# Stanford-ILIAD/PantheonRL

Measured on AMD Instinct MI355X. Metric: env-steps/sec (all agents) Overcooked-simple PPO self-play, higher is better.
Workload: dtype f32; 1 GPU; OvercookedMultiEnv-v0 layout=simple, PPO self-play (two independent PPO learners per GPU), synthetic (n_envs, n_steps, obs_dim) rollouts; n_envs=1024, n_steps=128, obs_dim=62, features=62, n_logits=6, batch_size=32768, n_epochs=10, agents_per_gpu=2, parallelism=2 agent(s) per gpu x1 gpu(s) = 2 learners (single process), launch_mode=graph, gemm_mode=2, action_masks=none, rollout=scripted, rollout_requested=scripted

## Files before the change

### include/pantheon_hip.h

```cpp
#ifndef PANTHEON_HIP_H
#define PANTHEON_HIP_H

#ifdef __cplusplus
extern "C" {
#endif

#define PH_ABI_VERSION 7
#define PH_HIDDEN 64
#define PH_MAX_COMP 256
#define PH_MAX_LOGITS 64
#define PH_MAX_BOX_ACT 16
#define PH_NSTAT 8
#define PH_MOD_MAX 8
#define PH_MAX_RANKS 16

#define PH_SPACE_BOX 0
#define PH_SPACE_DISCRETE 1

typedef struct ph_ctx ph_ctx;

typedef struct ph_space {
  int kind;
  int n;
  int nvec[PH_MAX_COMP];
// ... 30 lines not shown
  float clip_range;
  float clip_range_vf;
  float ent_coef;
  float vf_coef;
  float max_grad_norm;
  float target_kl;
  int normalize_advantage;
  float adam_beta1, adam_beta2, adam_eps;
} ph_ppo_hyper;

typedef struct ph_opt_state {
  float *params;
  float *adam_m;
  float *adam_v;
  int *step;
} ph_opt_state;

int ph_abi_version(void);
const char *ph_last_error(void);
int ph_device_count(int *n_out );
int ph_ctx_create(int device, ph_ctx **out );
int ph_ctx_destroy(ph_ctx *ctx);
int ph_ctx_set_stream(ph_ctx *ctx, void *hip_stream );
int ph_ctx_sync(ph_ctx *ctx);
int ph_graph_begin(ph_ctx *ctx);
int ph_graph_end(ph_ctx *ctx, int *graph_id_out );
int ph_graph_launch(ph_ctx *ctx, int graph_id);
int ph_ctx_set_rng_epoch(ph_ctx *ctx, unsigned long long *epoch_dev );
int ph_rng_epoch_advance(ph_ctx *ctx);
int ph_debug_set_profile_buffer(ph_ctx *ctx, long long *stamps_dev);
int ph_debug_weight_image_mismatches(ph_ctx *ctx, const ph_spec *spec, const float *params, int *mismatches);
int ph_set_exclusive_device(ph_ctx *ctx, int exclusive);
int ph_ctx_step_errors(ph_ctx *ctx, unsigned int *count_out );
int ph_timer_start(ph_ctx *ctx);
int ph_timer_stop(ph_ctx *ctx, float *ms_out );

int ph_layout_of(const ph_spec *spec , ph_layout *out );
int ph_debug_split_tables(const ph_spec *spec, int *slab_map, int *image_map, int *eligible);
int ph_debug_split_oh_tables(const ph_spec *spec, int *slab_map, int *image_map, int *slab_len_out, int *image_elems_out,
                             int *eligible);

int ph_buffer_add(ph_ctx *ctx, const ph_spec *spec, const ph_rollout *rb, int pos, const float *obs ,
                  const float *actions , const float *episode_start ,
                  const float *values , const float *log_probs );
int ph_buffer_add_reward(ph_ctx *ctx, const ph_rollout *rb, int pos, const float *reward ,
                         const unsigned char *env_mask );
int ph_buffer_add_reward_const(ph_ctx *ctx, const ph_rollout *rb, int pos, float reward);
#define PH_JOINT_MATCH_BONUS 0
#define PH_JOINT_RPS 1
int ph_ctx_set_joint_reward_rule(ph_ctx *ctx, int rule);

int ph_buffer_add_reward_joint(ph_ctx *ctx, const ph_rollout *rb, int pos, const float *base_reward ,
                               const int *joint_actions, int n_seats, int seat, const int *partner_seat ,
                               float bonus);
int ph_roundrobin_env_step(ph_ctx *ctx, const int *joint_actions, int *partnerid, const float *base_reward,
                           const float *done, float *reward_out, int *alt_action_out, float *next_block, int block_ld,
                           int n_partners, float bonus, int n);
typedef struct ph_rr_link {
  int n_partners, rank;
  int n, block_ld;
  void *area[PH_MAX_RANKS];
  unsigned long long *error;
  unsigned long long timeout_cycles;
} ph_rr_link;
typedef struct ph_rr_ego {
  const ph_spec *spec;
// ... 563 lines not shown
```

### pantheonrl_amd/_native.py

```python
from __future__ import annotations

import ctypes as C
import os
from typing import Optional, Sequence

PH_HIDDEN = 64
PH_MAX_COMP = 256
PH_MAX_LOGITS = 64
PH_MAX_BOX_ACT = 16
PH_NSTAT = 8
PH_SPACE_BOX = 0
PH_SPACE_DISCRETE = 1
STAT_NAMES = ("policy_loss", "value_loss", "entropy_loss", "clip_fraction", "approx_kl", "loss", "grad_norm", "applied")

_HERE = os.path.dirname(os.path.abspath(__file__))
LIB_PATH = os.environ.get("PANTHEON_HIP_LIB") or os.path.join(_HERE, "csrc", "libpantheon_hip.so")


class NativeError(RuntimeError):
    """Raised for any non-zero status from the C ABI (message from ph_last_error)."""


class PhSpace(C.Structure):
    _fields_ = [("kind", C.c_int), ("n", C.c_int), ("nvec", C.c_int * PH_MAX_COMP)]
# ... 238 lines not shown


SIGNATURES = {
    "ph_abi_version": [],
    "ph_roundrobin_env_step": [_vp, _vp, _vp, _vp, _vp, _vp, _vp, _vp, _i, _i, C.c_float, _i],
    "ph_last_error": [],
    "ph_device_count": [C.POINTER(_i)],
    "ph_ctx_create": [_i, C.POINTER(_vp)],
    "ph_ctx_destroy": [_vp],
    "ph_ctx_set_stream": [_vp, _vp],
    "ph_ctx_sync": [_vp],
    "ph_graph_begin": [_vp],
    "ph_graph_end": [_vp, C.POINTER(_i)],
    "ph_graph_launch": [_vp, _i],
    "ph_ctx_set_rng_epoch": [_vp, _vp],
    "ph_rng_epoch_advance": [_vp],
    "ph_debug_set_profile_buffer": [_vp, _vp],
    "ph_set_exclusive_device": [_vp, _i],
    "ph_ctx_step_errors": [_vp, C.POINTER(C.c_uint)],
    "ph_debug_weight_image_mismatches": [_vp, C.POINTER(PhSpec), _vp, C.POINTER(C.c_int)],
    "ph_timer_start": [_vp],
    "ph_timer_stop": [_vp, C.POINTER(C.c_float)],
    "ph_layout_of": [C.POINTER(PhSpec), C.POINTER(PhLayout)],
    "ph_debug_split_tables": [C.POINTER(PhSpec), C.POINTER(C.c_int), C.POINTER(C.c_int), C.POINTER(C.c_int)],
    "ph_debug_split_oh_tables": [C.POINTER(PhSpec), _vp, _vp, C.POINTER(_i), C.POINTER(_i), C.POINTER(_i)],
    "ph_buffer_add": [_vp, C.POINTER(PhSpec), C.POINTER(PhRollout), _i, _vp, _vp, _vp, _vp, _vp],
    "ph_buffer_add_reward": [_vp, C.POINTER(PhRollout), _i, _vp, _vp],
    "ph_buffer_add_reward_joint": [_vp, C.POINTER(PhRollout), _i, _vp, _vp, _i, _i, _vp, C.c_float],
    "ph_buffer_reset": [_vp, C.POINTER(PhSpec), C.POINTER(PhRollout)],
    "ph_gae": [_vp, C.POINTER(PhRollout), _vp, _vp, _d, _d, _i],
    "ph_policy_forward": [_vp, C.POINTER(PhSpec), _vp, _vp, _i, _vp, _vp, _vp, _ull, _ull, _i, _vp, _vp, _vp, _vp, _vp,
                          _vp, C.POINTER(PhRollout), _i, _vp, _vp, _i],
    "ph_ctx_set_joint_reward_rule": [_vp, _i],
    "ph_adapmult_layout_of": [C.POINTER(PhSpec), _i, _vp],
    "ph_adapmult_forward": [_vp, C.POINTER(PhSpec), _i, _vp, _vp, _i, _vp, _vp, _vp, _ull, _ull, _i, _vp, _vp, _vp, _vp, _vp,
                            _vp, C.POINTER(PhRollout), _i, _vp],
    "ph_adapmult_minibatch_grad": [_vp, C.POINTER(PhSpec), _i, _vp, C.POINTER(PhRollout), C.POINTER(PhPpoHyper), _vp, _i, _vp, _vp,
                                   _vp],
    "ph_adapmult_train": [_vp, C.POINTER(PhSpec), _i, C.POINTER(PhOptState), C.POINTER(PhRollout), C.POINTER(PhPpoHyper), _i, _i,
                          _vp, _ull, _vp, _vp],
    "ph_policy_act_host": [_vp, C.POINTER(PhSpec), _vp, _vp, _i, _vp, _ull, _ull, _i, _vp, _vp, _vp, C.POINTER(PhRollout), _i, _i],
    "ph_buffer_add_reward_const": [_vp, C.POINTER(PhRollout), _i, C.c_float],
    "ph_policy_step_multi": [_vp, _i, C.POINTER(PhStepCall)],
    "ph_policy_forward_ragged": [_vp, C.POINTER(PhSpec), _vp, _vp, _vp, _ull, _ull, _i, _vp, _vp, _vp, C.POINTER(PhRollout),
                                 _vp, _vp, _vp],
    "ph_buffer_add_reward_ragged": [_vp, C.POINTER(PhRollout), _vp, _vp, _vp],
    "ph_ragged_advance": [_vp, C.POINTER(PhRollout), _vp, _vp],
    "ph_buffer_compact_columns": [_vp, C.POINTER(PhSpec), C.POINTER(PhRollout), C.POINTER(PhRollout), _vp, _i],
    "ph_fix_illegal_actions": [_vp, _vp, _vp, _i, _i],
    "ph_rps_step": [_vp, _vp, _vp, _vp, _vp, _i],
    "ph_liar_step": [_vp, _vp, _vp, _vp, _vp, _vp, _vp, _vp, _vp, _vp, _i],
    "ph_liar_reset": [_vp, _vp, _vp, _vp, _vp, _vp, _ull, _ull, C.c_float, _i],
    "ph_liar_obs": [_vp, _vp, _vp, _vp, _vp, _vp, _vp, _i],
    "ph_liar_selfplay_step": [_vp, C.POINTER(PhLiarSelfPlay), _i, _ull, _i],
    "ph_liar_selfplay_rollout": [_vp, C.POINTER(PhLiarSelfPlay), _i, _i, _ull],
    "ph_pool_forward": [_vp, C.POINTER(PhSpec), C.POINTER(PhPoolMember), _i, _vp, _vp, _vp, _ull, _vp, _vp, _i],
    "ph_liar_default_actions": [_vp, _vp, _vp, _vp, _i],
    "ph_liar_pool_step": [_vp, C.POINTER(PhLiarPool), _i, _ull, _i],
    "ph_liar_xplay_step": [_vp, C.POINTER(PhLiarXplay), _ull, _i],
    "ph_xplay_stats": [_vp, _vp, _vp, _vp, _i, _i, _i, _vp],
    "ph_episode_stats": [_vp, C.POINTER(PhEpisodeScan)],
    "ph_liar_record_attach": [_vp, C.POINTER(PhLiarRecord)],
    "ph_liar_record_export": [_vp, C.POINTER(PhLiarRecord), _i, _vp, _vp, _vp, C.c_longlong],
    "ph_block_reset": [_vp, _i, _vp, _vp, _ull, _ull, _i],
    "ph_block_step": [_vp, _i, _vp, _vp, _i, _vp, _vp, _vp, _vp, _i],
    "ph_block_obs": [_vp, _i, _vp, _i, _vp, _vp, _i],
# ... 172 lines not shown
def adapmult_layout_of(spec: PhSpec, context_size: int) -> PhAdapMultLayout:
    lay = PhAdapMultLayout()
    check(load().ph_adapmult_layout_of(C.byref(spec), int(context_size), C.byref(lay)))
    return lay


def ptr(t) -> Optional[int]:
    if t is None:
        return None
    return t.data_ptr()


class Context:

    def __init__(self, device_index: int = 0):
        self.lib = load()
        h = C.c_void_p()
        check(self.lib.ph_ctx_create(int(device_index), C.byref(h)))
        self.handle = h
        self.device_index = int(device_index)
        self.exclusive_hint = False

    def set_stream(self, raw_stream: int) -> None:
        if raw_stream != getattr(self, "_bound_stream", None):
            check(self.lib.ph_ctx_set_stream(self.handle, C.c_void_p(raw_stream)))
            self._bound_stream = raw_stream

    def sync(self) -> None:
        check(self.lib.ph_ctx_sync(self.handle))

    def set_joint_reward_rule(self, rule: str) -> None:
        check(self.lib.ph_ctx_set_joint_reward_rule(self.handle, {"match": 0, "rps": 1}[rule]))

    def step_errors(self) -> int:
        n = C.c_uint(0)
        check(self.lib.ph_ctx_step_errors(self.handle, C.byref(n)))
        return int(n.value)

    def set_exclusive_device(self, exclusive: bool) -> None:
        check(self.lib.ph_set_exclusive_device(self.handle, int(bool(exclusive))))
        self.exclusive_hint = bool(exclusive)

    def close(self) -> None:
        if getattr(self, "handle", None):
            self.lib.ph_ctx_destroy(self.handle)
            self.handle = None

    def __del__(self):
        try:
            self.close()
        except Exception:
            pass


def feistel_indices(n: int, perm_seed: int, epoch: int, start: int = 0, count: Optional[int] = None):
    import numpy as np
    count = n - start if count is None else count
    out = (C.c_int * count)()
    check(load().ph_feistel_indices(int(n), int(perm_seed), int(epoch), int(start), int(count), out))
    return np.frombuffer(out, dtype=np.int32).copy()


def env_space_of(observation_space) -> PhSpace:
    kind = type(observation_space).__name__
    if kind == "Box":
        import numpy as np
# ... 51 lines not shown
```

### pantheonrl_amd/csrc/ph_abi.hip

```cpp
#include <dlfcn.h>
#include <hip/hip_runtime.h>
#include <rccl/rccl.h>

#include <atomic>
#include <chrono>
#include <cmath>
#include <cstdio>
#include <cstdint>
#include <cstring>
#include <mutex>
#include <string>
#include <vector>

#include "ph_launch.h"
#include "ph_block.h"
#include "ph_arch.h"
#include "ph_pool.h"
#include "ph_xplay.h"
#include "ph_record.h"
#include "ph_episode.h"
#include "ph_adap_vec.h"

namespace ph {

// ... 124 lines not shown
  float* am_buf = nullptr;
  size_t am_buf_cap = 0;
  float* adap_extra = nullptr;
  size_t adap_extra_cap = 0;
  float* adap_loss = nullptr;
  size_t adap_loss_cap = 0;
  float* scalars = nullptr;
  int* stop_flag = nullptr;
  std::vector<SpecCache> specs;
  std::vector<hipGraphExec_t> graphs;
  bool capturing = false;
  hipEvent_t ev0 = nullptr, ev1 = nullptr;
  ph_p2p* p2p_dev = nullptr;
  ph_p2p p2p_host;
  bool p2p_valid = false;
  void* comm = nullptr;
  int comm_world = 1, comm_rank = 0;
  hipEvent_t ev_grad = nullptr;
  int num_cu = 256;
  int exchange_blocks_per_cu = 0;
  unsigned long long* rng_epoch = nullptr;
  ph::RecordLog rec{};
  bool recording = false;
  ph::PoolMemberDev* pool_dev = nullptr;
  ph::PoolMemberDev pool_host[PH_MAX_POOL];
  int pool_count = 0;
  bool pool_wide = false;
  size_t pool_tower_lds = 0;
  int* pool_order = nullptr;
  size_t pool_order_cap = 0;
  int* pool_tiles = nullptr;
  size_t pool_tiles_cap = 0;
  long long* prof = nullptr;
  double* ep_partial = nullptr;
  size_t ep_partial_cap = 0;
  unsigned int* ep_ticket = nullptr;
  struct ModWs {
    float* act = nullptr;
    size_t act_cap = 0;
    int* maps = nullptr;
    ph_spec spec;
    ph_modular mod;
    bool maps_valid = false;
    float* kl_sum = nullptr;
    int* scratch = nullptr;
  } mw;
};

namespace {

struct DevGuard {
  int prev = -1;
  bool switched = false;
  explicit DevGuard(const ph_ctx* ctx) {
    if (!ctx) return;
    if (hipGetDevice(&prev) == hipSuccess && prev != ctx->device) switched = hipSetDevice(ctx->device) == hipSuccess;
  }
  ~DevGuard() {
    if (switched) (void)hipSetDevice(prev);
  }
  DevGuard(const DevGuard&) = delete;
  DevGuard& operator=(const DevGuard&) = delete;
};

template <typename T>
int ensure(const ph_ctx* ctx, T*& p, size_t& cap, size_t n) {
// ... 270 lines not shown
  a.prof = ctx->prof;
  a.deterministic = deterministic;
  fwd_bind_bases(a, rb, episode_start_in, pos_env, record_mask);
  PH_HIP(arch ? ph::launch_arch_fwd(a, ad, gemm_mode, ctx->stream) : ph::launch_policy_fwd(a, gemm_mode, ctx->stream));
  return 0;
}

int scripted_rollout_run(const char* who, ph_ctx* ctx, const ph_spec* spec, const ph_arch* arch, const float* params,
                         const float* obs_seq, const float* rew_seq, const float* done_seq, int n, int n_steps,
                         const float* episode_start0, unsigned long long seed, unsigned long long counter0, int* actions_i32,
                         float* values, float* log_probs, const ph_rollout* rb, int pos0, int gemm_mode) {
  if (!ctx) return fail("null ctx");
  if (!params || !obs_seq || !rew_seq || !done_seq || !episode_start0) return fail_who(who, ": null argument");
  if ((uintptr_t)params % 16 != 0) return fail_who(who, ": params must be 16-byte aligned");
  if (n <= 0 || n_steps <= 0) return fail_who(who, ": n and n_steps must be positive");
  if (check_rb(rb)) return 1;
  if (n != rb->E) return fail_who(who, ": n must equal the rollout buffer's E");
  if (pos0 < 0 || pos0 > rb->T - n_steps) return fail_who(who, ": rows pos0 .. pos0 + n_steps - 1 must lie in the buffer");
  ph::FwdArgs a;
  ph::ArchDims ad;
  if (fwd_args(a, ctx, spec, false, params, obs_seq, n, seed, counter0, actions_i32, values, log_probs, arch, &ad)) return 1;
  if (!arch && !ph::fwd16_eligible(a.nd, n))
    return fail_who(who, ": needs the 16-row forward's shape class (one feature chunk, one Discrete head of <= 8 logits, "
                         "n < 16384); use ph_policy_forward per step");
  a.prof = ctx->prof;
  if (fwd_bind_row(who, a, rb, pos0, episode_start0, nullptr)) return 1;
  ph::ScriptedSteps sc;
  std::memset(&sc, 0, sizeof(sc));
  sc.n_steps = n_steps;
  sc.obs_seq = obs_seq;
  sc.rew_seq = rew_seq;
  sc.done_seq = done_seq;
  PH_HIP(arch ? ph::launch_arch_rollout(a, ad, sc, gemm_mode, ctx->stream)
              : ph::launch_policy_fwd16_rollout(a, sc, gemm_mode, ctx->stream));
  return 0;
}

ph::AdvStatArgs adv_args_epochs(const ph_ctx* ctx, const ph_rollout* rb, const int* perms, unsigned long long perm_seed, int batch,
                                int n_mb) {
  const int N = rb->T * rb->E;
  ph::AdvStatArgs aa{};
  aa.rb_adv = rb->advantages;
  aa.T = rb->T;
  aa.E = rb->E;
  aa.perms = perms;
  aa.perm_n = (uint32_t)N;
  aa.perm_hb = ph::feistel_half_bits((uint32_t)N);
  aa.perm_seed = perm_seed;
  aa.epoch = ctx->rng_epoch;
  aa.N = N;
  aa.batch = batch;
  aa.n_mb = n_mb;
  aa.out = ctx->advstats;
  aa.partial = ctx->advpart;
  aa.idx_out = perms ? nullptr : ctx->perm_idx;
  aa.phys_out = ctx->perm_phys;
  return aa;
}
ph::AdvStatArgs adv_args_minibatch(const ph_ctx* ctx, const ph_rollout* rb, const int* indices, int nb) {
  ph::AdvStatArgs aa{};
  aa.rb_adv = rb->advantages;
  aa.T = rb->T;
  aa.E = rb->E;
  aa.perms = indices;
  aa.perm_hb = 1;
  aa.N = nb;
  aa.batch = nb;
// ... 150 lines not shown
}

int ph_ctx_destroy(ph_ctx* ctx) {
  DevGuard dev_guard(ctx);
  if (!ctx) return 0;
  (void)hipStreamSynchronize(ctx->stream);
  for (auto g : ctx->graphs)
    if (g) (void)hipGraphExecDestroy(g);
  for (auto& s : ctx->specs) {
    if (s.obs_off) (void)hipFree(s.obs_off);
    if (s.slab_map) (void)hipFree(s.slab_map);
    if (s.slab_map_split) (void)hipFree(s.slab_map_split);
    if (s.wimage_map) (void)hipFree(s.wimage_map);
    if (s.act_off) (void)hipFree(s.act_off);
  }
  void* ptrs[] = {ctx->wimage, ctx->mw.act, ctx->mw.maps, ctx->mw.kl_sum, ctx->mw.scratch, ctx->advpart, ctx->p2p_dev, ctx->slabs, ctx->statpart, ctx->grad, ctx->blocksq, ctx->advstats, ctx->adam_bias, ctx->perm_idx, ctx->perm_phys, ctx->ximg, ctx->rec_pi, ctx->rec_vf, ctx->rowrec, ctx->step_words, ctx->step_gen, ctx->scalars, ctx->stop_flag,
                  ctx->adap_extra, ctx->adap_loss, ctx->am_buf, ctx->pool_dev, ctx->pool_order, ctx->pool_tiles, ctx->ep_partial, ctx->ep_ticket};
  for (void* p : ptrs)
    if (p) (void)hipFree(p);
  if (ctx->act_stage_host) (void)hipHostFree(ctx->act_stage_host);
  if (ctx->act_done_host) (void)hipHostFree(ctx->act_done_host);
  if (ctx->ev0) (void)hipEventDestroy(ctx->ev0);
  if (ctx->ev1) (void)hipEventDestroy(ctx->ev1);
  if (ctx->ev_grad) (void)hipEventDestroy(ctx->ev_grad);
  (void)ph_comm_destroy(ctx);
  delete ctx;
  return 0;
}

int ph_ctx_set_joint_reward_rule(ph_ctx* ctx, int rule) {
  if (!ctx) return fail("null ctx");
  if (rule != PH_JOINT_MATCH_BONUS && rule != PH_JOINT_RPS) return fail("ph_ctx_set_joint_reward_rule: unknown rule");
  ctx->joint_reward_rule = rule;
  return 0;
}

int ph_ctx_set_stream(ph_ctx* ctx, void* hip_stream) {
  DevGuard dev_guard(ctx);
  if (!ctx) return fail("null ctx");
  ctx->stream = (hipStream_t)hip_stream;
  return 0;
}

int ph_ctx_sync(ph_ctx* ctx) {
  DevGuard dev_guard(ctx);
  if (!ctx) return fail("null ctx");
  PH_HIP(hipStreamSynchronize(ctx->stream));
  return 0;
}

int ph_graph_begin(ph_ctx* ctx) {
  DevGuard dev_guard(ctx);
  if (!ctx) return fail("null ctx");
  if (ctx->capturing) return fail("already capturing");
  if (ctx->stream == nullptr) return fail("graph capture needs a non-default stream (ph_ctx_set_stream)");
  PH_HIP(hipStreamBeginCapture(ctx->stream, hipStreamCaptureModeRelaxed));
  ctx->capturing = true;
  return 0;
}

int ph_graph_end(ph_ctx* ctx, int* graph_id_out) {
  DevGuard dev_guard(ctx);
  if (!ctx || !graph_id_out) return fail("null ctx/graph_id_out");
  if (!ctx->capturing) return fail("not capturing");
  ctx->capturing = false;
  hipGraph_t g = nullptr;
// ... 3076 lines not shown
```

### pantheonrl_amd/csrc/ph_launch.h

```cpp
#pragma once
#include "ph_device.h"

namespace ph {

__host__ __device__ inline unsigned p2p_stamp32(unsigned long long epoch, int T, int t) {
  return (unsigned)(epoch * (unsigned long long)T + (unsigned long long)t + 1ull);
}

__device__ __forceinline__ void p2p_note_timeout(unsigned long long* error, int kind, int t, unsigned long long index,
                                                 unsigned long long want, unsigned long long seen) {
  if (atomicAdd(error, 1ull) == 0ull) {
    error[1] = (unsigned long long)(unsigned)kind | ((unsigned long long)(unsigned)(t & 0xffffff) << 8) | (index << 32);
    error[2] = want;
    error[3] = seen;
  }
}

__device__ __forceinline__ void poll_backoff(int& polls) {
  if (polls < 16) __builtin_amdgcn_s_sleep(2);
  else if (polls < 64) __builtin_amdgcn_s_sleep(16);
  else __builtin_amdgcn_s_sleep(127);
  ++polls;
}

// ... 40 lines not shown
  const int* partner_seat;
  float bonus;
  int reward_rule;
  const unsigned char* env_mask;
  unsigned int* host_done;
  unsigned int host_seq;
};

struct ScriptedSteps {
  int n_steps;
  const float* obs_seq;
  const float* rew_seq;
  const float* done_seq;
  const unsigned char* mask_seq;
  int mask_policy, mask_env;
};

constexpr int MAX_LOCAL_AGENTS = 4;
struct P2PStep {
  const ph_p2p* x;
  int t;
  int a_local;
  int persistent;
};
__host__ __device__ inline int p2p_persistent_slot(unsigned long long epoch, int T, int t) { return (int)(epoch & 1ull) * T + t; }
struct FwdMulti {
  FwdArgs a[MAX_LOCAL_AGENTS];
  P2PStep px;
};
struct ScriptedMulti {
  ScriptedSteps sc[MAX_LOCAL_AGENTS];
};
bool fwd16_eligible(const NetDims& nd, int n);
hipError_t launch_policy_fwd16_rollout(const FwdArgs& a, const ScriptedSteps& sc, int gemm_mode, hipStream_t s);
hipError_t launch_policy_fwd16_exchange_rollout(const FwdMulti& m, const ScriptedMulti& sm, int n_agents, hipStream_t s);
hipError_t exchange_rollout_blocks_per_cu(int* blocks_out);

struct GradArgs {
  NetDims nd;
  const float* params;
  const float* rb_obs;
  const float* rb_act;
  const float* rb_val;
  const float* rb_logp;
  const float* rb_adv;
  const float* rb_ret;
  int T, E;
  const int* idx;
  const int* idx_phys;
  uint32_t perm_n, perm_hb;
  uint64_t perm_seed;
  int perm_epoch;
  const unsigned long long* epoch;
  int mb_start;
  int nb;
  const float* advstats;
  float clip, clip_vf, ent_coef, vf_coef;
  int norm_adv;
  float* slabs;
  float* statpart;
  const int* stop_flag;
  long long* prof;
  int ntiles;
  const unsigned short* wimage;
  const uint4* ximg;
  int ximg_zero_row;
  const uint4* rec_pi;
// ... 391 lines not shown
```

### pantheonrl_amd/csrc/ph_policy.hip

```cpp
#include <cstring>
#include <initializer_list>
#include "ph_rowtail.h"
#include "ph_liar_group.h"
#include "ph_pool.h"
#include "ph_bc_row.h"

namespace ph {


template <int R, int LP, bool VALU>
__device__ __forceinline__ void policy_fwd_body(const FwdArgs& a) {
  extern __shared__ __attribute__((aligned(16))) float smem[];
  constexpr int NT = R * 4;
  const NetDims& nd = a.nd;
  constexpr int Lp = LP, LDO = LP + 1;
  float* bufA = smem;
  float* bufB = bufA + R * LDH;
  float* w1s = bufB + R * LDH;
  float* w2s = w1s + HID * LDH;
  float* wos = w2s + HID * LDH;
  float* outs = wos + HID * LDO;
  float* b1s = outs + R * LDO;
  float* b2s = b1s + HID;
  float* bos = b2s + HID;
// ... 182 lines not shown
  __builtin_assume(a.rb_val != nullptr);
  __builtin_assume(a.rb_logp != nullptr);
  __builtin_assume(a.es_in != nullptr);
}
bool fwd_args_lean(const FwdArgs& a, bool joint_ok = false) {
  static int enabled = -1;
  if (enabled < 0) {
    const char* e = getenv("PH_ROLLOUT_LEAN");
    enabled = (e && e[0] == '0') ? 0 : 1;
  }
#ifdef PH_LEAN_PROF
  constexpr bool lean_prof = true;
#else
  constexpr bool lean_prof = false;
#endif
  return enabled && !a.mask && !a.uniforms && !a.given_actions && !a.deterministic && !a.act_f32 && !a.entropy && !a.logits && (lean_prof || !a.prof) &&
         !a.pos_env && !a.rec_mask && (joint_ok || (!a.joint && !a.joint_ll)) && !a.env_mask && !a.host_done && a.rb_obs && a.rb_act && a.rb_rew &&
         a.rb_es && a.rb_val && a.rb_logp && a.es_in;
}

constexpr int ZS_FLOATS = 4 * 16 * 8;

struct TailWaveHook {
  bool arrive, alive;
  long long* stamp;
  __device__ __forceinline__ void split(int act, float lse) const {
    if (stamp) stamp[4] = (long long)clock64();
    if (arrive) asm volatile("s_waitcnt lgkmcnt(0)\n\ts_barrier" ::"v"(act), "v"(lse) : "memory");
    else asm volatile("" ::"v"(act), "v"(lse));
  }
  __device__ __forceinline__ bool live() const { return alive; }
};

template <bool VALU, int LEAN = 0, int TW = 0>
__device__ __forceinline__ void policy_fwd16_body(const FwdArgs& a0, const ph_p2p* px = nullptr, int px_t = 0, int px_a_local = 0,
                                                  int agent = 0, const ScriptedSteps* sc = nullptr, int px_persistent = 0) {
  extern __shared__ __attribute__((aligned(16))) float smem[];
  constexpr int R = 16, NT = 256;
  const NetDims& nd = a0.nd;
  FwdArgs a = a0;
  if constexpr (LEAN == 1) fwd_args_pin_lean<false>(a);
  if constexpr (LEAN == 2) fwd_args_pin_lean<true>(a);
  if constexpr (TW != 0) {
    a.mask = nullptr;
    a.env_mask = nullptr;
    a.uniforms = nullptr;
    a.given_actions = nullptr;
    a.deterministic = 0;
  }
#ifdef PH_LEAN_PROF
  long long* const prof0 = a0.prof;
#else
  long long* const prof0 = LEAN ? nullptr : a0.prof;
#endif
  float* xs = smem;
  float* hs = xs + R * LDH;
  float* zs = hs + R * LDH;
  int* rowphys = (int*)(zs + ZS_FLOATS);
  float* upre = (float*)(rowphys + 16);
  unsigned long long** pxll = (unsigned long long**)(upre + 32);

  const int tid = threadIdx.x;
  const int wave = TW ? __builtin_amdgcn_readfirstlane(tid >> 6) : tid >> 6, lane = tid & 63, c = lane & 15, g = lane >> 4;
  const bool lw = TW == 0 || wave < 4;
  const int net = blockIdx.y;
  const int row0 = blockIdx.x * R;
  const ph_layout& lay = nd.lay;
  const float* W1 = a.params + (net == 0 ? lay.pi_W1 : lay.vf_W1);
  const float* B1 = a.params + (net == 0 ? lay.pi_b1 : lay.vf_b1);
  const float* W2 = a.params + (net == 0 ? lay.pi_W2 : lay.vf_W2);
  const float* B2 = a.params + (net == 0 ? lay.pi_b2 : lay.vf_b2);
  const int nk = nd.L;

  PH_STAMP(a.prof, 0);
  if (tid < R) rowphys[tid] = (row0 + tid < a.n) ? row0 + tid : -1;
  constexpr bool PXH = LEAN != 0;
  const int pxw_h = (PXH && px) ? px->world : 0, pxc_h = (PXH && px) ? px->count : 0, pxr_h = (PXH && px) ? px->rank : 0;
  const int pxT_h = (PXH && px) ? px->T : 1, pxslots_h = (PXH && px) ? px->ll_slots : 1;
  unsigned long long* const ll_self_h = (PXH && px) ? px->ll[pxr_h] : nullptr;
  if (PXH && px && tid < pxw_h && tid < PH_MAX_RANKS) pxll[tid] = px->ll[tid];
#define pxw (PXH ? pxw_h : px->world)
#define pxc (PXH ? pxc_h : px->count)
#define pxr (PXH ? pxr_h : px->rank)
#define pxT (PXH ? pxT_h : px->T)
#define pxslots (PXH ? pxslots_h : px->ll_slots)
#define ll_self (PXH ? ll_self_h : px->ll[px->rank])
#define PXLL(p) (PXH ? pxll[p] : px->ll[p])
  float bw1[16], bw2[16], bwh[4];
  const int col = 16 * wave + c;
#pragma unroll
  for (int s = 0; s < 16; ++s) {
    const int k = g + 4 * s;
    bw1[s] = (lw && k < nd.F) ? W1[k * HID + col] : 0.f;
    bw2[s] = lw ? W2[k * HID + col] : 0.f;
  }
#pragma unroll
  for (int s = 0; s < 4; ++s) {
    const int k = g + 4 * (4 * wave + s);
    bwh[s] = 0.f;
    if (!lw) continue;
    if (net == 0) {
      if (c < nk) bwh[s] = a.params[lay.act_W + k * nk + c];
    } else if (c == 0) {
      bwh[s] = a.params[lay.val_W + k];
    }
  }
  const float bias1 = lw ? B1[col] : 0.f, bias2 = lw ? B2[col] : 0.f;
  float hbias = 0.f;
  if (wave == 0) {
    if (net == 0) hbias = (c < nk) ? a.params[lay.act_b + c] : 0.f;
    else hbias = (c == 0) ? a.params[lay.val_b] : 0.f;
  }
  XStage<R, NT> xr;
  lds_only_barrier();
  if (sc) a.obs = sc->obs_seq;
  const bool xsync = nd.obs_kind != PH_SPACE_BOX;
  if (lw) xr.issue(rowphys, a.obs, nd, 0);
  const bool staged = sc != nullptr && nd.obs_kind == PH_SPACE_BOX;
  const bool copy_staged = staged && net == 1 && a.rb_obs && !a.pos_env && (TW ? wave != 0 && wave < 4 : wave != 0);
  const unsigned roff = RowStage3::base_offset(row0, nd, tid);
  RowStage3 rows;
  if (copy_staged) rows.issue(a.obs, a0.n, nd, roff, tid);
  if (lw) xr.commit(xs, rowphys, a.obs, nd, 0);
  if (TW != 0 && !lw && xsync) lds_only_barrier();
  vm_drain();
  if (copy_staged) rows.copy_out(a.rb_obs, a0.n, nd.D, roff, tid);
  lds_only_barrier();
  PH_STAMP(a.prof, 1);

  const int n_steps = sc ? sc->n_steps : 1;
  unsigned long long epoch_hi = 0ull;
  if (sc) {
    epoch_hi = a0.epoch ? (unsigned long long)(*a0.epoch) << 32 : 0ull;
    a.epoch = nullptr;
    a.counter = a0.counter + epoch_hi;
  }
  const unsigned long long px_epoch = (px && px_persistent) ? *px->epoch : 0ull;
  const bool draw_ahead = sc && net == 0 && !a.uniforms && !a.deterministic && !a.given_actions;
  auto draw_uniforms = [&](int t1) {
    if (lane < R && row0 + lane < a0.n)
      upre[(t1 & 1) * R + lane] = philox_uniform(a0.seed, a0.counter + (unsigned long long)t1 + epoch_hi, (uint32_t)(row0 + lane), 0u);
  };
  if (TW == 0 && draw_ahead && wave == 1) draw_uniforms(0);

  auto product = [&](const float* A, const float (&bw)[16]) -> f32x4 {
    f32x4 e = {0.f, 0.f, 0.f, 0.f}, o = {0.f, 0.f, 0.f, 0.f};
    const float* ap = A + c * LDH + g;
    float av[16];
#pragma unroll
    for (int s = 0; s < 16; ++s) av[s] = ap[4 * s];
    __builtin_amdgcn_sched_barrier(0);
#pragma unroll
    for (int s = 0; s < 16; s += 2) {
      e = mma16<VALU>(av[s], bw[s], e, lane);
      o = mma16<VALU>(av[s + 1], bw[s + 1], o, lane);
    }
    return e + o;
  };

  auto step_record = [&](FwdArgs& a, int t) {
    const size_t row = (size_t)t * a0.n;
    a.obs = sc->obs_seq + row * nd.D;
    a.counter = a0.counter + (unsigned long long)t + epoch_hi;
    a.rb_obs = a0.rb_obs + row * nd.D;
    a.rb_act = a0.rb_act + row * nd.A;
    a.rb_rew = a0.rb_rew + row;
    a.rb_es = a0.rb_es + row;
    a.rb_val = a0.rb_val + row;
// ... 25 lines not shown
#pragma unroll
      for (int h = 0; h < 2; ++h) {
        z[4 * h + 0] = (q[0][h].x + q[1][h].x) + (q[2][h].x + q[3][h].x);
        z[4 * h + 1] = (q[0][h].y + q[1][h].y) + (q[2][h].y + q[3][h].y);
        z[4 * h + 2] = (q[0][h].z + q[1][h].z) + (q[2][h].z + q[3][h].z);
        z[4 * h + 3] = (q[0][h].w + q[1][h].w) + (q[2][h].w + q[3][h].w);
      }
    }
    if (net == 0) {
      const uint64_t ctr = fwd_counter(a);
      int act;
      switch (nk) {
        case 1: act = discrete8_row_tail<1>(a, nd, grow, z, ctr, up, pstep, hook); break;
        case 2: act = discrete8_row_tail<2>(a, nd, grow, z, ctr, up, pstep, hook); break;
        case 3: act = discrete8_row_tail<3>(a, nd, grow, z, ctr, up, pstep, hook); break;
        case 4: act = discrete8_row_tail<4>(a, nd, grow, z, ctr, up, pstep, hook); break;
        case 5: act = discrete8_row_tail<5>(a, nd, grow, z, ctr, up, pstep, hook); break;
        case 6: act = discrete8_row_tail<6>(a, nd, grow, z, ctr, up, pstep, hook); break;
        case 7: act = discrete8_row_tail<7>(a, nd, grow, z, ctr, up, pstep, hook); break;
        default: act = discrete8_row_tail<8>(a, nd, grow, z, ctr, up, pstep, hook); break;
      }
      if (px && hook.live()) {
        const int pt = px_t + t;
        const int slot = px_persistent ? p2p_persistent_slot(px_epoch, pxT, pt) : pt % pxslots;
        const size_t off = (size_t)slot * pxw * pxc + (size_t)(pxr * px_a_local + agent) * a.n + grow;
        const unsigned long long w =
            ((unsigned long long)p2p_stamp32(px_persistent ? px_epoch : *px->epoch, pxT, pt) << 32) | (unsigned long long)(unsigned)act;
        for (int p = 0; p < pxw; ++p)
          __hip_atomic_store(PXLL(p) + off, w, __ATOMIC_RELAXED, __HIP_MEMORY_SCOPE_SYSTEM);
      }
    } else {
      if (hook.live()) {
        value_row_tail(a, grow, z[0], !a.pos_env && a.rb_val, vpre);
        if (sc && t == n_steps - 1) {
          float add = sc->rew_seq[(size_t)t * a0.n + grow];
          if (px_persistent && a0.joint) {
            FwdArgs b = a;
            b.joint_ll = ll_self + (size_t)p2p_persistent_slot(px_epoch, pxT, t) * pxw * pxc;
            b.ll_t = t;
            int p = *a0.partner_seat;
            p = p < 0 ? 0 : (p >= a0.n_seats ? a0.n_seats - 1 : p);
            const int mine = ll_read(b, b.joint_ll + (size_t)a0.seat * a0.n + grow);
            const int theirs = ll_read(b, b.joint_ll + (size_t)p * a0.n + grow);
            add += joint_reward(mine, theirs, a0.bonus, a0.reward_rule);
          }
          a.rb_rew[grow] += add;
        }
      }
      hook.split(0, z[0]);
    }
  };

  if constexpr (TW != 0) {
    if (!lw) {
      const int nlive = (a0.n - row0 < R) ? a0.n - row0 : R;
      const int r = lane < nlive ? lane : nlive - 1, grow = row0 + r;
      const bool live = lane < nlive;
#ifdef PH_LEAN_PROF
      long long* const wstamp = (prof0 && lane == 0) ? prof0 + ((size_t)blockIdx.y * gridDim.x + blockIdx.x) * 16 : nullptr;
#else
      long long* const wstamp = nullptr;
#endif
      auto draw = [&](int t) { return philox_uniform(a0.seed, a0.counter + (unsigned long long)t + epoch_hi, (uint32_t)grow, 0u); };
      auto preload = [&](const FwdArgs& a) {
        return (net == 1 && !a.pos_env && a.rb_val) ? value_row_preload(a, grow) : ValuePre{0.f, 0.f, 0.f, 0ull, 0ull, 0u, 0, 0};
      };
      if (draw_ahead) upre[r] = draw(0);
      ValuePre vpre = preload(a);
      lds_only_barrier();
      lds_only_barrier();
      lds_only_barrier();
      for (int s = 0; s < n_steps; ++s) {
        const bool more = s + 1 < n_steps;
        if (more) {
          if (xsync) lds_only_barrier();
          lds_only_barrier();
        }
        long long* const ws = (s == 7) ? wstamp : nullptr;
        if (ws) ws[2] = (long long)clock64();
        row_tail(a, s, r, grow, vpre, draw_ahead ? upre + r : nullptr, nullptr, TailWaveHook{more, live, ws});
        if (ws) ws[6] = (long long)clock64();
        if (more) {
          step_record(a, s + 1);
          vpre = preload(a);
          lds_only_barrier();
          if (draw_ahead) upre[r] = draw(s + 1);
          lds_only_barrier();
        }
      }
      return;
    }
    __builtin_amdgcn_s_setprio(1);
  }

  for (int t = 0; t < n_steps; ++t) {
  long long* const pstep = (sc && t == 8) ? prof0 : nullptr;
  PH_STAMP(pstep, 8);
  if (t > 0) {
    step_record(a, t);
    if (!staged) {
      xr.issue(rowphys, a.obs, nd, 0);
      xr.commit(xs, rowphys, a.obs, nd, 0);
      vm_drain();
    }
    lds_only_barrier();
  }
  PH_STAMP(pstep, 9);
  const bool more = t + 1 < n_steps;
  const float* const obs_next = sc ? sc->obs_seq + (size_t)(t + 1) * a0.n * nd.D : nullptr;
  if (TW != 0 && staged && more && wave != 0) rows.issue(obs_next, a0.n, nd, roff, tid);

  const bool pre_ok = TW == 0 && net == 1 && wave == 0 && lane < R && row0 + lane < a.n && !a.pos_env && a.rb_val;
  ValuePre vpre = {0.f, 0.f, 0.f, 0ull, 0ull, 0u, 0, 0};
  if (pre_ok) vpre = value_row_preload(a, row0 + lane);
  const bool copy_from_regs = net == 1 && a.rb_obs && !a.pos_env && nd.obs_kind == PH_SPACE_BOX;
  {
    const f32x4 z1 = product(xs, bw1);
#pragma unroll
    for (int r = 0; r < 4; ++r) hs[(4 * g + r) * LDH + col] = fast_tanh(z1[r] + bias1);
  }
  lds_only_barrier();
  PH_STAMP(a.prof, 3);
  PH_STAMP(pstep, 10);
  {
    const f32x4 z2 = product(hs, bw2);
#pragma unroll
    for (int r = 0; r < 4; ++r) xs[(4 * g + r) * LDH + col] = fast_tanh(z2[r] + bias2);
  }
  lds_only_barrier();
  PH_STAMP(a.prof, 5);
  PH_STAMP(pstep, 11);

  if (TW == 0 && staged && net == 1 && more && wave != 0) rows.issue(obs_next, a0.n, nd, roff, tid);

  {
    if (wave == 0 && pre_ok) value_row_preload_words(a, row0 + lane, vpre);
    const float* ap = xs + c * LDH + g + 16 * wave;
    float av[4];
#pragma unroll
    for (int j = 0; j < 4; ++j) av[j] = ap[4 * j];
    f32x4 e = {0.f, 0.f, 0.f, 0.f}, o = {0.f, 0.f, 0.f, 0.f};
// ... 40 lines not shown
      }
    }
  } else if (net == 1) {
    copy_obs_rows(a, row0, (a.n - row0 < R) ? a.n - row0 : R, nd.D, TW ? tid : -1, NT);
  }
  PH_STAMP(a.prof, 7);
  PH_STAMP(pstep, 15);
  }
}

#undef pxw
#undef pxc
#undef pxr
#undef pxT
#undef pxslots
#undef ll_self
#undef PXLL

template <bool VALU, bool LEAN = false>
__global__ __launch_bounds__(256) void policy_fwd16_kernel(FwdArgs a) {
  policy_fwd16_body<VALU, LEAN ? 1 : 0>(a);
  if constexpr (!LEAN) {
    if (a.host_done) {
      __threadfence_system();
      __syncthreads();
      if (threadIdx.x == 0) __hip_atomic_store(a.host_done + blockIdx.y, a.host_seq, __ATOMIC_RELEASE, __HIP_MEMORY_SCOPE_SYSTEM);
    }
  }
}
constexpr int ROLLOUT_THREADS = 320;
template <bool VALU, bool LEAN>
__global__ __launch_bounds__(VALU ? 256 : ROLLOUT_THREADS) void policy_fwd16_rollout_kernel(FwdArgs a, ScriptedSteps sc) {
  policy_fwd16_body<VALU, LEAN ? 1 : 0, VALU ? 0 : 4>(a, nullptr, 0, 0, 0, &sc);
}
template <bool LEAN>
__global__ __launch_bounds__(256) void policy_fwd16_multi_kernel(FwdMulti m) {
  policy_fwd16_body<false, LEAN ? 2 : 0>(m.a[blockIdx.z], m.px.x, m.px.t, m.px.a_local, blockIdx.z);
}
template <bool LEAN>
__global__ __launch_bounds__(256, 3) void policy_fwd16_exchange_rollout_kernel(FwdMulti m, ScriptedMulti sm) {
  policy_fwd16_body<false, LEAN ? 2 : 0>(m.a[blockIdx.z], m.px.x, 0, m.px.a_local, blockIdx.z, &sm.sc[blockIdx.z], 1);
}

static size_t fwd16_lds_bytes() { return sizeof(float) * (size_t)(2 * 16 * LDH + ZS_FLOATS + 16 + 32) + sizeof(void*) * PH_MAX_RANKS; }

bool fwd16_eligible(const NetDims& nd, int n) {
  static int enabled = -1;
  if (enabled < 0) {
    const char* e = getenv("PH_FWD16");
    enabled = (e && e[0] == '0') ? 0 : 1;
  }
  return enabled && !nd.gauss && nd.nchunk == 1 && nd.A == 1 && nd.L <= 8 && n < 16384;
}

template <bool VALU>
static hipError_t launch_fwd16_variant(const FwdArgs& a, hipStream_t s) {
  const size_t lds = fwd16_lds_bytes();
  const bool general = VALU || !fwd_args_lean(a);
  const void* fn = general ? (const void*)policy_fwd16_kernel<VALU> : (const void*)policy_fwd16_kernel<false, true>;
  if (const hipError_t e = allow_dynamic_lds(fn, lds); e != hipSuccess) return e;
  if (general) hipLaunchKernelGGL((policy_fwd16_kernel<VALU>), dim3((a.n + 15) / 16, 2), dim3(256), lds, s, a);
  else hipLaunchKernelGGL((policy_fwd16_kernel<false, true>), dim3((a.n + 15) / 16, 2), dim3(256), lds, s, a);
  return hipGetLastError();
}

static size_t rollout_lds_bytes(int nwg_total) {
  const int cu = device_cu_count();
  return (cu > 0 && 2 * nwg_total <= cu) ? (size_t)81 * 1024 + 512 : fwd16_lds_bytes();
}
hipError_t launch_policy_fwd16_rollout(const FwdArgs& a, const ScriptedSteps& sc, int gemm_mode, hipStream_t s) {
  if (a.mask || a.env_mask || a.uniforms || a.given_actions || a.deterministic || sc.mask_seq) return hipErrorInvalidValue;
  const int variant = gemm_mode == 1 ? 1 : (fwd_args_lean(a) ? 2 : 0);
  dim3 grid((a.n + 15) / 16, 2), block(variant == 1 ? 256 : ROLLOUT_THREADS);
  const size_t lds = rollout_lds_bytes((int)(grid.x * grid.y));
  const void* fn = variant == 1 ? (const void*)policy_fwd16_rollout_kernel<true, false>
                                : (variant == 2 ? (const void*)policy_fwd16_rollout_kernel<false, true> : (const void*)policy_fwd16_rollout_kernel<false, false>);
  if (const hipError_t e = allow_dynamic_lds(fn, lds); e != hipSuccess) return e;
  if (variant == 1) hipLaunchKernelGGL((policy_fwd16_rollout_kernel<true, false>), grid, block, lds, s, a, sc);
  else if (variant == 2) hipLaunchKernelGGL((policy_fwd16_rollout_kernel<false, true>), grid, block, lds, s, a, sc);
  else hipLaunchKernelGGL((policy_fwd16_rollout_kernel<false, false>), grid, block, lds, s, a, sc);
  return hipGetLastError();
}

hipError_t exchange_rollout_blocks_per_cu(int* blocks_out) {
  const size_t lds = fwd16_lds_bytes();
  int api = 0;
  hipError_t e = hipOccupancyMaxActiveBlocksPerMultiprocessor(&api, (const void*)policy_fwd16_exchange_rollout_kernel<false>, 256, lds);
  if (e != hipSuccess) return e;
  const int by_lds = (int)((size_t)160 * 1024 / lds);
  int blocks = api < 8 ? api : 8;
  if (blocks > by_lds) blocks = by_lds;
  else if (blocks < by_lds && blocks > 1) blocks -= 1;
  *blocks_out = blocks < 1 ? 1 : blocks;
  return hipSuccess;
}

hipError_t launch_policy_fwd16_exchange_rollout(const FwdMulti& m, const ScriptedMulti& sm, int n_agents, hipStream_t s) {
  bool lean = true;
  for (int i = 0; i < n_agents; ++i) lean = lean && fwd_args_lean(m.a[i], true) && !sm.sc[i].mask_seq;
  const dim3 grid((m.a[0].n + 15) / 16, 2, n_agents);
  if (lean) hipLaunchKernelGGL(policy_fwd16_exchange_rollout_kernel<true>, grid, dim3(256), fwd16_lds_bytes(), s, m, sm);
  else hipLaunchKernelGGL(policy_fwd16_exchange_rollout_kernel<false>, grid, dim3(256), fwd16_lds_bytes(), s, m, sm);
  return hipGetLastError();
}

// ... 1082 lines not shown
```

Before: 129.0 million agent-steps/s.

## Split scripted rollout across time chunks in parallel grid z-dimension

Adds a chunked rollout kernel that splits the n_steps time loop into independent chunks launched along grid z. Scripted observations and done flags are precomputed, so each chunk can start from its own offset in the rollout buffer. An automatic heuristic picks the chunk count from the CU count and workgroup count, aiming to fill an under-occupied GPU (n=1024 gives only 128 workgroups). The cost is redundant per-chunk setup, use of the smaller LDS configuration, and a changed RNG counter per chunk.

```diff
diff --git a/include/pantheon_hip.h b/include/pantheon_hip.h
--- a/include/pantheon_hip.h
+++ b/include/pantheon_hip.h
@@ -86,6 +86,8 @@
 int ph_debug_weight_image_mismatches(ph_ctx *ctx, const ph_spec *spec, const float *params, int *mismatches);
 int ph_set_exclusive_device(ph_ctx *ctx, int exclusive);
 int ph_ctx_step_errors(ph_ctx *ctx, unsigned int *count_out );
+int ph_ctx_set_rollout_chunks(ph_ctx *ctx, int chunks);
+int ph_ctx_rollout_chunks(ph_ctx *ctx, int n, int n_steps, int *chunks_out );
 int ph_timer_start(ph_ctx *ctx);
 int ph_timer_stop(ph_ctx *ctx, float *ms_out );
 
diff --git a/pantheonrl_amd/_native.py b/pantheonrl_amd/_native.py
--- a/pantheonrl_amd/_native.py
+++ b/pantheonrl_amd/_native.py
@@ -294,6 +294,8 @@
     "ph_policy_forward": [_vp, C.POINTER(PhSpec), _vp, _vp, _i, _vp, _vp, _vp, _ull, _ull, _i, _vp, _vp, _vp, _vp, _vp,
                           _vp, C.POINTER(PhRollout), _i, _vp, _vp, _i],
     "ph_ctx_set_joint_reward_rule": [_vp, _i],
+    "ph_ctx_set_rollout_chunks": [_vp, _i],
+    "ph_ctx_rollout_chunks": [_vp, _i, _i, C.POINTER(_i)],
     "ph_adapmult_layout_of": [C.POINTER(PhSpec), _i, _vp],
     "ph_adapmult_forward": [_vp, C.POINTER(PhSpec), _i, _vp, _vp, _i, _vp, _vp, _vp, _ull, _ull, _i, _vp, _vp, _vp, _vp, _vp,
                             _vp, C.POINTER(PhRollout), _i, _vp],
@@ -532,6 +534,14 @@
     def set_joint_reward_rule(self, rule: str) -> None:
         check(self.lib.ph_ctx_set_joint_reward_rule(self.handle, {"match": 0, "rps": 1}[rule]))
 
+    def set_rollout_chunks(self, chunks: int) -> None:
+        check(self.lib.ph_ctx_set_rollout_chunks(self.handle, int(chunks)))
+
+    def rollout_chunks(self, n: int, n_steps: int) -> int:
+        k = C.c_int(0)
+        check(self.lib.ph_ctx_rollout_chunks(self.handle, int(n), int(n_steps), C.byref(k)))
+        return int(k.value)
+
     def step_errors(self) -> int:
         n = C.c_uint(0)
         check(self.lib.ph_ctx_step_errors(self.handle, C.byref(n)))
diff --git a/pantheonrl_amd/csrc/ph_abi.hip b/pantheonrl_amd/csrc/ph_abi.hip
--- a/pantheonrl_amd/csrc/ph_abi.hip
+++ b/pantheonrl_amd/csrc/ph_abi.hip
@@ -180,6 +180,7 @@
   int* pool_tiles = nullptr;
   size_t pool_tiles_cap = 0;
   long long* prof = nullptr;
+  int rollout_chunks = 0;
   double* ep_partial = nullptr;
   size_t ep_partial_cap = 0;
   unsigned int* ep_ticket = nullptr;
@@ -516,7 +517,7 @@
   sc.rew_seq = rew_seq;
   sc.done_seq = done_seq;
   PH_HIP(arch ? ph::launch_arch_rollout(a, ad, sc, gemm_mode, ctx->stream)
-              : ph::launch_policy_fwd16_rollout(a, sc, gemm_mode, ctx->stream));
+              : ph::launch_policy_fwd16_rollout(a, sc, gemm_mode, ctx->stream, ctx->rollout_chunks));
   return 0;
 }
 
@@ -733,6 +734,20 @@
   if (!ctx) return fail("null ctx");
   if (rule != PH_JOINT_MATCH_BONUS && rule != PH_JOINT_RPS) return fail("ph_ctx_set_joint_reward_rule: unknown rule");
   ctx->joint_reward_rule = rule;
+  return 0;
+}
+
+int ph_ctx_set_rollout_chunks(ph_ctx* ctx, int chunks) {
+  if (!ctx) return fail("null ctx");
+  if (chunks < 0) return fail("ph_ctx_set_rollout_chunks: chunks must be 0 (automatic), 1 (serial) or a forced count");
+  ctx->rollout_chunks = chunks;
+  return 0;
+}
+int ph_ctx_rollout_chunks(ph_ctx* ctx, int n, int n_steps, int* chunks_out) {
+  DevGuard dev_guard(ctx);
+  if (!ctx || !chunks_out) return fail("ph_ctx_rollout_chunks: null argument");
+  if (n <= 0 || n_steps <= 0) return fail("ph_ctx_rollout_chunks: n and n_steps must be positive");
+  *chunks_out = ph::rollout_chunk_count(n, n_steps, ctx->rollout_chunks);
   return 0;
 }
 
diff --git a/pantheonrl_amd/csrc/ph_launch.h b/pantheonrl_amd/csrc/ph_launch.h
--- a/pantheonrl_amd/csrc/ph_launch.h
+++ b/pantheonrl_amd/csrc/ph_launch.h
@@ -96,7 +96,8 @@
   ScriptedSteps sc[MAX_LOCAL_AGENTS];
 };
 bool fwd16_eligible(const NetDims& nd, int n);
-hipError_t launch_policy_fwd16_rollout(const FwdArgs& a, const ScriptedSteps& sc, int gemm_mode, hipStream_t s);
+hipError_t launch_policy_fwd16_rollout(const FwdArgs& a, const ScriptedSteps& sc, int gemm_mode, hipStream_t s, int chunks = 0);
+int rollout_chunk_count(int n, int n_steps, int chunks);
 hipError_t launch_policy_fwd16_exchange_rollout(const FwdMulti& m, const ScriptedMulti& sm, int n_agents, hipStream_t s);
 hipError_t exchange_rollout_blocks_per_cu(int* blocks_out);
 
diff --git a/pantheonrl_amd/csrc/ph_policy.hip b/pantheonrl_amd/csrc/ph_policy.hip
--- a/pantheonrl_amd/csrc/ph_policy.hip
+++ b/pantheonrl_amd/csrc/ph_policy.hip
@@ -238,15 +238,36 @@
   __device__ __forceinline__ bool live() const { return alive; }
 };
 
-template <bool VALU, int LEAN = 0, int TW = 0>
+template <bool VALU, int LEAN = 0, int TW = 0, bool CH = false>
 __device__ __forceinline__ void policy_fwd16_body(const FwdArgs& a0, const ph_p2p* px = nullptr, int px_t = 0, int px_a_local = 0,
-                                                  int agent = 0, const ScriptedSteps* sc = nullptr, int px_persistent = 0) {
+                                                  int agent = 0, const ScriptedSteps* sc = nullptr, int px_persistent = 0,
+                                                  int ch_lo = 0, int ch_hi = 0) {
+  static_assert(!CH || (TW == 4 && !VALU), "chunks: the tail-wave form of the one-launch rollout");
   extern __shared__ __attribute__((aligned(16))) float smem[];
   constexpr int R = 16, NT = 256;
   const NetDims& nd = a0.nd;
   FwdArgs a = a0;
   if constexpr (LEAN == 1) fwd_args_pin_lean<false>(a);
   if constexpr (LEAN == 2) fwd_args_pin_lean<true>(a);
+  if constexpr (CH) {
+    if (ch_lo > 0) {
+      const size_t row = (size_t)ch_lo * a0.n;
+      a.rb_obs = a0.rb_obs + row * nd.D;
+      a.rb_act = a0.rb_act + row * nd.A;
+      a.rb_rew = a0.rb_rew + row;
+      a.rb_es = a0.rb_es + row;
+      a.rb_val = a0.rb_val + row;
+      a.rb_logp = a0.rb_logp + row;
+      a.es_in = sc->done_seq + (row - a0.n);
+    }
+    if (ch_hi != sc->n_steps) {
+      a.act_i32 = nullptr;
+      a.values = nullptr;
+      a.logp = nullptr;
+    }
+    const int ps = sc->n_steps > 8 ? 8 : sc->n_steps - 1;
+    if (ps < ch_lo || ps >= ch_hi) a.prof = nullptr;
+  }
   if constexpr (TW != 0) {
     a.mask = nullptr;
     a.env_mask = nullptr;
@@ -255,9 +276,9 @@
     a.deterministic = 0;
   }
 #ifdef PH_LEAN_PROF
-  long long* const prof0 = a0.prof;
+  long long* const prof0 = CH ? a.prof : a0.prof;
 #else
-  long long* const prof0 = LEAN ? nullptr : a0.prof;
+  long long* const prof0 = LEAN ? nullptr : (CH ? a.prof : a0.prof);
 #endif
   float* xs = smem;
   float* hs = xs + R * LDH;
@@ -319,7 +340,8 @@
   }
   XStage<R, NT> xr;
   lds_only_barrier();
-  if (sc) a.obs = sc->obs_seq;
+  if constexpr (CH) a.obs = sc->obs_seq + (size_t)ch_lo * a0.n * nd.D;
+  else if (sc) a.obs = sc->obs_seq;
   const bool xsync = nd.obs_kind != PH_SPACE_BOX;
   if (lw) xr.issue(rowphys, a.obs, nd, 0);
   const bool staged = sc != nullptr && nd.obs_kind == PH_SPACE_BOX;
@@ -335,11 +357,13 @@
   PH_STAMP(a.prof, 1);
 
   const int n_steps = sc ? sc->n_steps : 1;
+  const int t_lo = CH ? ch_lo : 0, t_hi = CH ? ch_hi : n_steps;
   unsigned long long epoch_hi = 0ull;
   if (sc) {
     epoch_hi = a0.epoch ? (unsigned long long)(*a0.epoch) << 32 : 0ull;
     a.epoch = nullptr;
     a.counter = a0.counter + epoch_hi;
+    if constexpr (CH) a.counter += (unsigned long long)ch_lo;
   }
   const unsigned long long px_epoch = (px && px_persistent) ? *px->epoch : 0ull;
   const bool draw_ahead = sc && net == 0 && !a.uniforms && !a.deterministic && !a.given_actions;
@@ -431,7 +455,7 @@
     } else {
       if (hook.live()) {
         value_row_tail(a, grow, z[0], !a.pos_env && a.rb_val, vpre);
-        if (sc && t == n_steps - 1) {
+        if (sc && t == t_hi - 1) {
           float add = sc->rew_seq[(size_t)t * a0.n + grow];
           if (px_persistent && a0.joint) {
             FwdArgs b = a;
@@ -443,7 +467,13 @@
             const int theirs = ll_read(b, b.joint_ll + (size_t)p * a0.n + grow);
             add += joint_reward(mine, theirs, a0.bonus, a0.reward_rule);
           }
-          a.rb_rew[grow] += add;
+          if constexpr (CH) {
+            float zero = 0.f;
+            asm volatile("" : "+v"(zero));
+            a.rb_rew[grow] = zero + add;
+          } else {
+            a.rb_rew[grow] += add;
+          }
         }
       }
       hook.split(0, z[0]);
@@ -464,13 +494,13 @@
       auto preload = [&](const FwdArgs& a) {
         return (net == 1 && !a.pos_env && a.rb_val) ? value_row_preload(a, grow) : ValuePre{0.f, 0.f, 0.f, 0ull, 0ull, 0u, 0, 0};
       };
-      if (draw_ahead) upre[r] = draw(0);
+      if (draw_ahead) upre[r] = draw(t_lo);
       ValuePre vpre = preload(a);
       lds_only_barrier();
       lds_only_barrier();
       lds_only_barrier();
-      for (int s = 0; s < n_steps; ++s) {
-        const bool more = s + 1 < n_steps;
+      for (int s = t_lo; s < t_hi; ++s) {
+        const bool more = s + 1 < t_hi;
         if (more) {
           if (xsync) lds_only_barrier();
           lds_only_barrier();
@@ -492,10 +522,10 @@
     __builtin_amdgcn_s_setprio(1);
   }
 
-  for (int t = 0; t < n_steps; ++t) {
+  for (int t = t_lo; t < t_hi; ++t) {
   long long* const pstep = (sc && t == 8) ? prof0 : nullptr;
   PH_STAMP(pstep, 8);
-  if (t > 0) {
+  if (t > t_lo) {
     step_record(a, t);
     if (!staged) {
       xr.issue(rowphys, a.obs, nd, 0);
@@ -505,7 +535,7 @@
     lds_only_barrier();
   }
   PH_STAMP(pstep, 9);
-  const bool more = t + 1 < n_steps;
+  const bool more = t + 1 < t_hi;
   const float* const obs_next = sc ? sc->obs_seq + (size_t)(t + 1) * a0.n * nd.D : nullptr;
   if (TW != 0 && staged && more && wave != 0) rows.issue(obs_next, a0.n, nd, roff, tid);
 
@@ -612,6 +642,13 @@
 template <bool VALU, bool LEAN>
 __global__ __launch_bounds__(VALU ? 256 : ROLLOUT_THREADS) void policy_fwd16_rollout_kernel(FwdArgs a, ScriptedSteps sc) {
   policy_fwd16_body<VALU, LEAN ? 1 : 0, VALU ? 0 : 4>(a, nullptr, 0, 0, 0, &sc);
+}
+template <bool LEAN>
+__global__ __launch_bounds__(ROLLOUT_THREADS) void policy_fwd16_rollout_chunk_kernel(FwdArgs a, ScriptedSteps sc, int base, int rem) {
+  const int z = (int)blockIdx.z;
+  const int lo = z * base + (z < rem ? z : rem), hi = lo + base + (z < rem ? 1 : 0);
+  if (lo >= hi || hi > sc.n_steps) return;
+  policy_fwd16_body<false, LEAN ? 1 : 0, 4, true>(a, nullptr, 0, 0, 0, &sc, 0, lo, hi);
 }
 template <bool LEAN>
 __global__ __launch_bounds__(256) void policy_fwd16_multi_kernel(FwdMulti m) {
@@ -648,9 +685,36 @@
   const int cu = device_cu_count();
   return (cu > 0 && 2 * nwg_total <= cu) ? (size_t)81 * 1024 + 512 : fwd16_lds_bytes();
 }
-hipError_t launch_policy_fwd16_rollout(const FwdArgs& a, const ScriptedSteps& sc, int gemm_mode, hipStream_t s) {
+constexpr int ROLLOUT_CHUNK_MIN_STEPS = 16, ROLLOUT_CHUNK_WG_NUM = 3, ROLLOUT_CHUNK_CU_DEN = 2;
+int rollout_chunk_count(int n, int n_steps, int forced) {
+  if (n_steps < 1) return 1;
+  static int env_forced = -1;
+  if (env_forced < 0) {
+    const char* e = getenv("PH_ROLLOUT_CHUNKS");
+    env_forced = (e && e[0] >= '0' && e[0] <= '9') ? atoi(e) : 0;
+  }
+  if (forced < 1) forced = env_forced;
+#ifdef PH_LEAN_PROF
+  if (forced < 1) forced = 1;
+#endif
+  if (forced >= 1) return forced < n_steps ? forced : n_steps;
+  const int cu = device_cu_count(), nwg = 2 * ((n + 15) / 16);
+  if (cu <= 0) return 1;
+  int c = (ROLLOUT_CHUNK_WG_NUM * cu + ROLLOUT_CHUNK_CU_DEN * nwg - 1) / (ROLLOUT_CHUNK_CU_DEN * nwg);
+  if (c > n_steps / ROLLOUT_CHUNK_MIN_STEPS) c = n_steps / ROLLOUT_CHUNK_MIN_STEPS;
+  return c < 1 ? 1 : c;
+}
+hipError_t launch_policy_fwd16_rollout(const FwdArgs& a, const ScriptedSteps& sc, int gemm_mode, hipStream_t s, int chunks) {
   if (a.mask || a.env_mask || a.uniforms || a.given_actions || a.deterministic || sc.mask_seq) return hipErrorInvalidValue;
   const int variant = gemm_mode == 1 ? 1 : (fwd_args_lean(a) ? 2 : 0);
+  const int nchunk = variant == 1 ? 1 : rollout_chunk_count(a.n, sc.n_steps, chunks);
+  if (nchunk > 1) {
+    const dim3 cgrid((a.n + 15) / 16, 2, nchunk);
+    const int base = sc.n_steps / nchunk, rem = sc.n_steps - base * nchunk;
+    if (variant == 2) hipLaunchKernelGGL((policy_fwd16_rollout_chunk_kernel<true>), cgrid, dim3(ROLLOUT_THREADS), fwd16_lds_bytes(), s, a, sc, base, rem);
+    else hipLaunchKernelGGL((policy_fwd16_rollout_chunk_kernel<false>), cgrid, dim3(ROLLOUT_THREADS), fwd16_lds_bytes(), s, a, sc, base, rem);
+    return hipGetLastError();
+  }
   dim3 grid((a.n + 15) / 16, 2), block(variant == 1 ? 256 : ROLLOUT_THREADS);
   const size_t lds = rollout_lds_bytes((int)(grid.x * grid.y));
   const void* fn = variant == 1 ? (const void*)policy_fwd16_rollout_kernel<true, false>
```

Measured after the change: 130.8 million agent-steps/s (median of 6 runs). Within noise of the previous version (+1.4%).
